# TaWeiTu/vp8

Hardware: NVIDIA B200
Metric: decoded 1080p frames/s (higher is better)
Workload: dtype u8

## Files before the change

vp8_b200/csrc/cuda/recon_kernels.cu:

```cuda
#include "recon_kernels.h"

#include <algorithm>
#include <cstring>

namespace vp8r {

__constant__ int c_taps[2][8][2];
__constant__ int c_taps6[2][8][6];
__constant__ unsigned short c_bpred_lut[10 * 16];

static int PackTaps(int a, int b, int c, int d) {
  return (a & 0xff) | ((b & 0xff) << 8) | ((c & 0xff) << 16) | ((d & 0xff) << 24);
}

static void BuildBpredLut(unsigned short *lut) {
  auto L = [](int k) { return 3 - k; };
  auto A = [](int k) { return 5 + k; };
  const int P = 4;
  auto put3 = [&](int mode, int y, int x, int a, int b, int c) {
    lut[mode * 16 + y * 4 + x] = (unsigned short)(a | (b << 4) | (c << 8) | (0 << 12));
  };
  auto put2 = [&](int mode, int y, int x, int a, int c) {
    lut[mode * 16 + y * 4 + x] = (unsigned short)(a | (a << 4) | (c << 8) | (1 << 12));
  };
// ... 20 lines not shown
  put3(7, 3, 3, A(5), A(6), A(7));
  put2(8, 3, 0, 0, 1);    put3(8, 3, 1, 0, 1, 2); put2(8, 2, 0, 1, 2);    put2(8, 3, 2, 1, 2);
  put3(8, 2, 1, 1, 2, 3); put3(8, 3, 3, 1, 2, 3); put2(8, 2, 2, 2, 3);    put2(8, 1, 0, 2, 3);
  put3(8, 2, 3, 2, 3, 4); put3(8, 1, 1, 2, 3, 4); put2(8, 1, 2, 3, 4);    put2(8, 0, 0, 3, 4);
  put3(8, 1, 3, 3, 4, 5); put3(8, 0, 1, 3, 4, 5); put3(8, 0, 2, 4, 5, 6); put3(8, 0, 3, 5, 6, 7);
  put2(9, 0, 0, L(0), L(1));       put3(9, 0, 1, L(0), L(1), L(2)); put2(9, 0, 2, L(1), L(2));
  put2(9, 1, 0, L(1), L(2));       put3(9, 0, 3, L(1), L(2), L(3)); put3(9, 1, 1, L(1), L(2), L(3));
  put2(9, 1, 2, L(2), L(3));       put2(9, 2, 0, L(2), L(3));       put3(9, 1, 3, L(2), L(3), L(3));
  put3(9, 2, 1, L(2), L(3), L(3));
  put3(9, 2, 2, L(3), L(3), L(3)); put3(9, 2, 3, L(3), L(3), L(3)); put3(9, 3, 0, L(3), L(3), L(3));
  put3(9, 3, 1, L(3), L(3), L(3)); put3(9, 3, 2, L(3), L(3), L(3)); put3(9, 3, 3, L(3), L(3), L(3));
}

cudaError_t InitKernelTables() {
  static const int six[8][6] = {{0, 0, 128, 0, 0, 0},  {0, -6, 123, 12, -1, 0},   {2, -11, 108, 36, -8, 1},
                                {0, -9, 93, 50, -6, 0}, {3, -16, 77, 77, -16, 3}, {0, -6, 50, 93, -9, 0},
                                {1, -8, 36, 108, -11, 2}, {0, -1, 12, 123, -6, 0}};
  int taps[2][8][2];
  for (int f = 0; f < 8; ++f) {
    taps[0][f][0] = PackTaps(six[f][0], six[f][1], six[f][2], six[f][3]);
    taps[0][f][1] = PackTaps(six[f][4], six[f][5], 0, 0);
    taps[1][f][0] = PackTaps(0, 0, 128 - 16 * f, 16 * f);
    taps[1][f][1] = 0;
  }
  cudaError_t err = cudaMemcpyToSymbol(c_taps, taps, sizeof(taps));
  if (err != cudaSuccess) return err;
  int taps6[2][8][6];
  for (int f = 0; f < 8; ++f)
    for (int k = 0; k < 6; ++k) {
      taps6[0][f][k] = six[f][k];
      taps6[1][f][k] = k == 2 ? 128 - 16 * f : (k == 3 ? 16 * f : 0);
    }
  err = cudaMemcpyToSymbol(c_taps6, taps6, sizeof(taps6));
  if (err != cudaSuccess) return err;
  err = InitParseTables();
  if (err != cudaSuccess) return err;
  unsigned short lut[160];
  std::memset(lut, 0, sizeof(lut));
  BuildBpredLut(lut);
  err = InitEncodeTables(lut);
  if (err != cudaSuccess) return err;
  return cudaMemcpyToSymbol(c_bpred_lut, lut, sizeof(lut));
}

__device__ __forceinline__ int dp4a_us(unsigned a, int b, int c) {
  int d;
  asm("dp4a.u32.s32 %0, %1, %2, %3;" : "=r"(d) : "r"(a), "r"(b), "r"(c));
  return d;
}
__device__ __forceinline__ int clamp255(int x) { return min(max(x, 0), 255); }
__device__ __forceinline__ int clamp128(int x) { return min(max(x, -128), 127); }
__device__ __forceinline__ int s16(int x) { return (int)(short)x; }

__device__ __forceinline__ void Idct4x4(int *m) {
#pragma unroll
  for (int i = 0; i < 4; ++i) {
    int a = m[i] + m[8 + i], b = m[i] - m[8 + i];
    int t1 = (m[4 + i] * 35468) >> 16;
    int t2 = m[12 + i] + ((m[12 + i] * 20091) >> 16);
    int c = t1 - t2;
    t1 = m[4 + i] + ((m[4 + i] * 20091) >> 16);
    t2 = (m[12 + i] * 35468) >> 16;
    int d = t1 + t2;
    m[i] = s16(a + d);
    m[12 + i] = s16(a - d);
    m[4 + i] = s16(b + c);
    m[8 + i] = s16(b - c);
  }
#pragma unroll
  for (int i = 0; i < 4; ++i) {
    int *r = m + 4 * i;
    int a = r[0] + r[2], b = r[0] - r[2];
    int t1 = (r[1] * 35468) >> 16;
    int t2 = r[3] + ((r[3] * 20091) >> 16);
    int c = t1 - t2;
    t1 = r[1] + ((r[1] * 20091) >> 16);
    t2 = (r[3] * 35468) >> 16;
    int d = t1 + t2;
    r[0] = s16((a + d + 4) >> 3);
    r[3] = s16((a - d + 4) >> 3);
    r[1] = s16((b + c + 4) >> 3);
    r[2] = s16((b - c + 4) >> 3);
  }
}

__device__ __forceinline__ void Iwht4x4(int *m) {
#pragma unroll
  for (int i = 0; i < 4; ++i) {
    int a = m[i] + m[12 + i], b = m[4 + i] + m[8 + i];
    int c = m[4 + i] - m[8 + i], d = m[i] - m[12 + i];
    m[i] = s16(a + b);
    m[4 + i] = s16(c + d);
    m[8 + i] = s16(a - b);
    m[12 + i] = s16(d - c);
  }
#pragma unroll
  for (int i = 0; i < 4; ++i) {
    int *r = m + 4 * i;
    int a = r[0] + r[3], b = r[1] + r[2];
    int c = r[1] - r[2], d = r[0] - r[3];
    r[0] = s16((a + b + 3) >> 3);
    r[1] = s16((c + d + 3) >> 3);
    r[2] = s16((a - b + 3) >> 3);
    r[3] = s16((d - c + 3) >> 3);
  }
}

__device__ __forceinline__ bool WarpResidual(const DevFrameJob &job, const vp8r_mb_info &mb, int lane,
                                            short *y2_slot, int *res) {
  const unsigned mask = mb.coef_mask;
  if (mask == 0) return false;
  const bool has_y2 = (mb.flags & VP8R_MB_HAS_Y2) != 0;
  const int blk = lane < 24 ? lane + 1 : 0;
  const bool coded = lane <= 24 && ((mask >> blk) & 1);
  const int16_t *dq = job.dq[(mb.flags >> VP8R_MB_QSEG_SHIFT) & 3];
#pragma unroll
  for (int i = 0; i < 16; ++i) res[i] = 0;
  if (coded) {
    const int at = __popc(mask & ((1u << blk) - 1));
    const int4 *src = reinterpret_cast<const int4 *>(job.payload + (size_t)(mb.coef_offset + at) * 16);
    int4 lo = __ldg(src), hi = __ldg(src + 1);
    int w[8] = {lo.x, lo.y, lo.z, lo.w, hi.x, hi.y, hi.z, hi.w};
    int dc = blk == 0 ? dq[VP8R_DQ_Y2_DC] : (blk <= 16 ? dq[VP8R_DQ_Y1_DC] : dq[VP8R_DQ_UV_DC]);
    int ac = blk == 0 ? dq[VP8R_DQ_Y2_AC] : (blk <= 16 ? dq[VP8R_DQ_Y1_AC] : dq[VP8R_DQ_UV_AC]);
#pragma unroll
    for (int i = 0; i < 8; ++i) {
      res[2 * i] = s16(s16(w[i]) * ac);
      res[2 * i + 1] = s16((w[i] >> 16) * ac);
    }
    res[0] = s16(s16(w[0]) * dc);
  }
  bool any = coded;
  if (has_y2 && (mask & 1)) {
    if (lane == 24) {
      Iwht4x4(res);
#pragma unroll
      for (int i = 0; i < 16; ++i) y2_slot[i] = (short)res[i];
    }
    __syncwarp();
    if (lane < 16) {
      res[0] = y2_slot[lane];
      any = true;
    }
    __syncwarp();
  }
  if (lane < 24 && any) Idct4x4(res);
  return lane < 24 && any;
}

__device__ __forceinline__ unsigned Filter4(unsigned lo, unsigned mid, unsigned hi, int t03, int t45) {
  unsigned out = 0;
#pragma unroll
  for (int j = 0; j < 4; ++j) {
    unsigned a = j ? __funnelshift_r(lo, mid, 8 * j) : lo;
    unsigned b = j ? __funnelshift_r(mid, hi, 8 * j) : mid;
    int s = dp4a_us(a, t03, 64);
    s = dp4a_us(b, t45, s);
    out |= (unsigned)clamp255(s >> 7) << (8 * j);
  }
  return out;
}

__device__ __forceinline__ void Transpose4x4(unsigned r0, unsigned r1, unsigned r2, unsigned r3, unsigned &c0,
                                             unsigned &c1, unsigned &c2, unsigned &c3) {
  unsigned t0 = __byte_perm(r0, r1, 0x5140), t1 = __byte_perm(r2, r3, 0x5140);
  unsigned t2 = __byte_perm(r0, r1, 0x7362), t3 = __byte_perm(r2, r3, 0x7362);
  c0 = __byte_perm(t0, t1, 0x5410);
  c1 = __byte_perm(t0, t1, 0x7632);
  c2 = __byte_perm(t2, t3, 0x5410);
  c3 = __byte_perm(t2, t3, 0x7632);
}

__device__ __forceinline__ unsigned PackSat4(int o0, int o1, int o2, int o3) {
  unsigned t, d;
  asm("cvt.pack.sat.u8.s32.b32 %0, %1, %2, %3;" : "=r"(t) : "r"(o3), "r"(o2), "r"(0));
  asm("cvt.pack.sat.u8.s32.b32 %0, %1, %2, %3;" : "=r"(d) : "r"(o1), "r"(o0), "r"(t));
  return d;
}

__device__ __forceinline__ unsigned Filter4P(unsigned lo, unsigned mid, unsigned hi, int t03, int t45) {
  int s[4];
#pragma unroll
  for (int j = 0; j < 4; ++j) {
    unsigned a = j ? __funnelshift_r(lo, mid, 8 * j) : lo;
    unsigned b = j ? __funnelshift_r(mid, hi, 8 * j) : mid;
    s[j] = dp4a_us(b, t45, dp4a_us(a, t03, 64)) >> 7;
  }
  return PackSat4(s[0], s[1], s[2], s[3]);
}

struct TapsAt {
  int lo1, lo2, lo3, mid1, mid2, mid3, hi3;
};
__device__ __forceinline__ TapsAt MakeTapsAt(int t03, int t45) {
  TapsAt t;
  t.lo1 = t03 << 8; t.lo2 = t03 << 16; t.lo3 = t03 << 24;
  t.mid1 = (int)__funnelshift_l((unsigned)t03, (unsigned)t45, 8);
  t.mid2 = (int)__funnelshift_l((unsigned)t03, (unsigned)t45, 16);
  t.mid3 = (int)__funnelshift_l((unsigned)t03, (unsigned)t45, 24);
  t.hi3 = (int)((unsigned)t45 >> 8);
  return t;
}
__device__ __forceinline__ unsigned Filter4T(unsigned lo, unsigned mid, unsigned hi, int t03, int t45, const TapsAt &t) {
  const int s0 = dp4a_us(mid, t45, dp4a_us(lo, t03, 64)) >> 7;
  const int s1 = dp4a_us(mid, t.mid1, dp4a_us(lo, t.lo1, 64)) >> 7;
  const int s2 = dp4a_us(mid, t.mid2, dp4a_us(lo, t.lo2, 64)) >> 7;
  const int s3 = dp4a_us(hi, t.hi3, dp4a_us(mid, t.mid3, dp4a_us(lo, t.lo3, 64))) >> 7;
  return PackSat4(s0, s1, s2, s3);
}

__device__ __forceinline__ unsigned Vert6(const unsigned *e, const unsigned *o, const int *t) {
  const unsigned bias = (8192u + 64u) * 0x00010001u;
  unsigned ae = bias, ao = bias;
#pragma unroll
  for (int k = 0; k < 6; ++k) {
    ae += (unsigned)t[k] * e[k];
    ao += (unsigned)t[k] * o[k];
  }
  ae = (ae >> 7) & 0x01ff01ffu;
  ao = (ao >> 7) & 0x01ff01ffu;
  ae = __vmins2(__viaddmax_s16x2(ae, 0xffc0ffc0u, 0u), 0x00ff00ffu);
  ao = __vmins2(__viaddmax_s16x2(ao, 0xffc0ffc0u, 0u), 0x00ff00ffu);
  return ae | (ao << 8);
// ... 23 lines not shown
      "MBAR_WAIT_%=:\n\t"
      "mbarrier.try_wait.parity.shared::cta.b64 p, [%0], %1;\n\t"
      "@p bra MBAR_DONE_%=;\n\t"
      "bra MBAR_WAIT_%=;\n\t"
      "MBAR_DONE_%=:\n\t}" ::"r"(SmemAddr(bar)), "r"(parity)
      : "memory");
}
__device__ __forceinline__ void TmaLoad2D(void *dst, const DevTensorMap *map, int x, int y, unsigned long long *bar) {
  asm volatile("cp.async.bulk.tensor.2d.shared::cluster.global.mbarrier::complete_tx::bytes [%0], [%1, {%2, %3}], [%4];" ::"r"(
                   SmemAddr(dst)),
               "l"(map), "r"(x), "r"(y), "r"(SmemAddr(bar))
               : "memory");
}

struct __align__(128) InterTile {
  unsigned char luma[kTmaLumaBoxH * kTmaLumaBoxW];
  unsigned char pad0[1024 - kTmaLumaBoxH * kTmaLumaBoxW];
  unsigned char cu[kTmaChromaBoxH * kTmaChromaBoxW];
  unsigned char pad1[640 - kTmaChromaBoxH * kTmaChromaBoxW];
  unsigned char cv[kTmaChromaBoxH * kTmaChromaBoxW];
  unsigned char pad2[640 - kTmaChromaBoxH * kTmaChromaBoxW - 8];
  unsigned long long bar;
};
static_assert(sizeof(InterTile) == 2304, "tile layout");
constexpr unsigned kInterTileTxBytes = kTmaLumaBoxH * kTmaLumaBoxW + 2 * kTmaChromaBoxH * kTmaChromaBoxW;

struct WholeMbGeometry {
  int fr, fc, cfr, cfc;
  int wy, wx, cwy, cwx;
};
__device__ __forceinline__ WholeMbGeometry WholeGeometry(const DevFrameJob &job, const vp8r_mb_info &mb, int mb_r, int mb_c) {
  WholeMbGeometry g;
  const int mvr = mb.mv[0], mvc = mb.mv[1];
  const int sr = s16(4 * mvr), sc = s16(4 * mvc);
  const int ar = (abs(sr) + 4) >> 3, ac = (abs(sc) + 4) >> 3;
  int cmr = sr < 0 ? -ar : ar, cmc = sc < 0 ? -ac : ac;
  if (job.version == 3) {
    cmr &= ~7;
    cmc &= ~7;
  }
  g.fr = mvr & 7; g.fc = mvc & 7; g.cfr = cmr & 7; g.cfc = cmc & 7;
  g.wy = min(max(mb_r * 16 + (mvr >> 3) - 2, -kBorder), job.mb_rows * 16 + kBorder - 21);
  g.wx = min(max(mb_c * 16 + (mvc >> 3) - 2, -kBorder), job.mb_cols * 16 + kBorder - 21);
  g.cwy = min(max(mb_r * 8 + (cmr >> 3) - 2, -kBorder), job.mb_rows * 8 + kBorder - 13);
  g.cwx = min(max(mb_c * 8 + (cmc >> 3) - 2, -kBorder), job.mb_cols * 8 + kBorder - 13);
  return g;
}

struct __align__(16) InterScratch {
  unsigned hl[23 * 4];
  unsigned hc[2][13 * 2];
  short res[24][16];
  short y2[16];
};

template <bool kTma>
__device__ __forceinline__ void InterMacroblockWhole(const DevFrameJob &job, const vp8r_mb_info &mb, int mb_r, int mb_c,
                                                     int lane, InterScratch &s, bool has_res, const WholeMbGeometry &g,
                                                     InterTile *tile) {
  const int ref_id = (mb.flags >> VP8R_MB_REF_SHIFT) & 3;
  const int bil = job.version != 0;
  const int fr = g.fr, fc = g.fc, cfr = g.cfr, cfc = g.cfc;

  if (kTma) {
    MbarWait(&tile->bar, 0);
    {
      const int dx = (g.wx + kBorder) & 15;
      const int w = lane & 3, row0 = lane >> 2, base = (dx >> 2) + w;
      const unsigned shift = (dx & 3) * 8;
      const int r_lo = fr ? 0 : 2, r_hi = (fr | fc) ? (fr ? 21 : 18) : 0;
      const int t03 = c_taps[bil][fc][0], t45 = c_taps[bil][fc][1];
      const TapsAt ta = MakeTapsAt(t03, t45);
#pragma unroll
      for (int k = 0; k < 3; ++k) {
        const int row = row0 + 8 * k;
        if (row >= r_lo && row < r_hi) {
          const unsigned *p = reinterpret_cast<const unsigned *>(tile->luma + row * kTmaLumaBoxW) + base;
          const unsigned w0 = p[0], w1 = p[1], w2 = p[2];
          const unsigned lo = __funnelshift_r(w0, w1, shift), mid = __funnelshift_r(w1, w2, shift), hi = w2 >> shift;
          s.hl[HlRow(row) + w] = fc ? Filter4T(lo, mid, hi, t03, t45, ta) : __funnelshift_r(lo, mid, 16);
        }
      }
    }
    {
      const int dx = (g.cwx + kBorder) & 15;
      const int row = lane >> 1, cw_ = lane & 1, base = (dx >> 2) + cw_;
      const unsigned shift = (dx & 3) * 8;
      const int r_lo = cfr ? 0 : 2, r_hi = (cfr | cfc) ? (cfr ? 13 : 10) : 0;
      const int t03 = c_taps[bil][cfc][0], t45 = c_taps[bil][cfc][1];
      const TapsAt ta = MakeTapsAt(t03, t45);
      if (row >= r_lo && row < r_hi) {
#pragma unroll
        for (int pl = 0; pl < 2; ++pl) {
          const unsigned *p = reinterpret_cast<const unsigned *>((pl ? tile->cv : tile->cu) + row * kTmaChromaBoxW) + base;
          const unsigned w0 = p[0], w1 = p[1], w2 = p[2];
          const unsigned lo = __funnelshift_r(w0, w1, shift), mid = __funnelshift_r(w1, w2, shift), hi = w2 >> shift;
          s.hc[pl][row * 2 + cw_] = cfc ? Filter4T(lo, mid, hi, t03, t45, ta) : __funnelshift_r(lo, mid, 16);
        }
      }
    }
  } else
  {
    const int pitch = job.pitch_y, cpitch = job.pitch_c;
    const int wy = g.wy, wx = g.wx;
    const uint8_t *wp = job.ref[ref_id].y + (ptrdiff_t)wy * pitch + wx;
    const unsigned shift = ((unsigned)(size_t)wp & 3u) * 8;
// ... 62 lines not shown
      out1 = Vert6(e + 1, o + 1, t);
    } else if (kTma && fc == 0) {
      const int dx2 = ((g.wx + kBorder) & 15) + 2;
      const unsigned *p = reinterpret_cast<const unsigned *>(tile->luma + (y0 + 2) * kTmaLumaBoxW) + (dx2 >> 2) + w;
      const unsigned sh = (dx2 & 3) * 8;
      out0 = __funnelshift_r(p[0], p[1], sh);
      out1 = __funnelshift_r(p[kTmaLumaBoxW / 4], p[kTmaLumaBoxW / 4 + 1], sh);
    } else {
      out0 = s.hl[HlRow(y0 + 2) + w];
      out1 = s.hl[HlRow(y0 + 3) + w];
    }
    if (has_res) {
      const uint2 *rp = reinterpret_cast<const uint2 *>(&s.res[(y0 >> 2) * 4 + w][(y0 & 3) * 4]);
      const uint2 ra = rp[0], rb = rp[1];
      out0 = AddResidual4(out0, ra.x, ra.y);
      out1 = AddResidual4(out1, rb.x, rb.y);
    }
    uint8_t *d = job.cur.y + (ptrdiff_t)(mb_r * 16 + y0) * job.pitch_y + mb_c * 16 + 4 * w;
    *reinterpret_cast<unsigned *>(d) = out0;
    *reinterpret_cast<unsigned *>(d + job.pitch_y) = out1;
  }
  {
    const int pl = lane >> 4, y = (lane >> 1) & 7, w = lane & 1;
    const unsigned *h = s.hc[pl];
    unsigned out;
    if (cfr) {
      unsigned e[6], o[6];
#pragma unroll
      for (int k = 0; k < 6; ++k) {
        const unsigned r = h[(y + k) * 2 + w];
        e[k] = __byte_perm(r, 0, 0x4240);
        o[k] = __byte_perm(r, 0, 0x4341);
      }
      out = Vert6(e, o, c_taps6[bil][cfr]);
    } else if (kTma && cfc == 0) {
      const int dx2 = ((g.cwx + kBorder) & 15) + 2;
      const unsigned *p = reinterpret_cast<const unsigned *>((pl ? tile->cv : tile->cu) + (y + 2) * kTmaChromaBoxW) + (dx2 >> 2) + w;
      out = __funnelshift_r(p[0], p[1], (dx2 & 3) * 8);
    } else {
      out = h[(y + 2) * 2 + w];
    }
    if (has_res) {
      const uint2 ra = *reinterpret_cast<const uint2 *>(&s.res[16 + pl * 4 + (y >> 2) * 2 + w][(y & 3) * 4]);
      out = AddResidual4(out, ra.x, ra.y);
    }
    uint8_t *d = (pl ? job.cur.v : job.cur.u) + (ptrdiff_t)(mb_r * 8 + y) * job.pitch_c + mb_c * 8 + 4 * w;
    *reinterpret_cast<unsigned *>(d) = out;
  }
}

constexpr int kInterWarps = 4;

#ifndef VP8R_INTER_MINBLOCKS
#define VP8R_INTER_MINBLOCKS 12
#endif
template <bool kTma>
__device__ __forceinline__ void InterOneMacroblock(const DevFrameJob &job, int mb_r, int mb_c, int lane, InterScratch &scratch, InterTile *tile) {
  const int mb_index = mb_r * job.mb_cols + mb_c;
  vp8r_mb_info mb;
  {
    const int4 *p = reinterpret_cast<const int4 *>(job.mbs + mb_index);
    int4 a = __ldg(p), b = __ldg(p + 1);
    mb.flags = a.x; mb.coef_mask = a.y; mb.coef_offset = a.z;
    mb.mv[0] = (short)(a.w & 0xffff); mb.mv[1] = (short)(a.w >> 16);
    mb.aux[0] = b.x; mb.aux[1] = b.y;
  }
  if (!(mb.flags & VP8R_MB_IS_INTER)) return;

  const bool split = ((mb.flags >> VP8R_MB_MODE_SHIFT) & 7) == 4;
  WholeMbGeometry geo{};
  if (!split) {
    geo = WholeGeometry(job, mb, mb_r, mb_c);
    if (kTma && lane == 0) {
      const DevTensorMap *maps = job.ref_tmap[(mb.flags >> VP8R_MB_REF_SHIFT) & 3];
      MbarExpectTx(&tile->bar, kInterTileTxBytes);
      TmaLoad2D(tile->luma, maps + 0, (geo.wx + kBorder) & ~15, geo.wy + kBorder, &tile->bar);
      TmaLoad2D(tile->cu, maps + 1, (geo.cwx + kBorder) & ~15, geo.cwy + kBorder, &tile->bar);
      TmaLoad2D(tile->cv, maps + 2, (geo.cwx + kBorder) & ~15, geo.cwy + kBorder, &tile->bar);
    }
  }
  int res[16];
  const bool has_res = WarpResidual(job, mb, lane, scratch.y2, res);
  if (!split) {
    const bool mb_has_res = mb.coef_mask != 0;
    if (mb_has_res && lane < 24) {
      uint4 *dst = reinterpret_cast<uint4 *>(scratch.res[lane]);
#pragma unroll
      for (int q = 0; q < 2; ++q) {
        unsigned v[4];
#pragma unroll
        for (int i = 0; i < 4; ++i) {
          const int a = has_res ? res[8 * q + 2 * i] : 0, b = has_res ? res[8 * q + 2 * i + 1] : 0;
          v[i] = ((unsigned)a & 0xffffu) | ((unsigned)b << 16);
        }
        dst[q] = make_uint4(v[0], v[1], v[2], v[3]);
      }
    }
    InterMacroblockWhole<kTma>(job, mb, mb_r, mb_c, lane, scratch, mb_has_res, geo, tile);
    return;
  }
  if (lane >= 24) return;

  const int ref_id = (mb.flags >> VP8R_MB_REF_SHIFT) & 3;
  const int *split_mv = reinterpret_cast<const int *>(job.payload + (size_t)mb.aux[0] * 16);

  int mvr, mvc, bx, by, pitch, plane_w, plane_h;
  const uint8_t *ref;
  uint8_t *dst;
  if (lane < 16) {
    int m = split ? __ldg(split_mv + lane) : (int)((unsigned short)mb.mv[0] | ((unsigned)(unsigned short)mb.mv[1] << 16));
    mvr = (short)(m & 0xffff);
    mvc = m >> 16;
    by = mb_r * 16 + (lane >> 2) * 4;
    bx = mb_c * 16 + (lane & 3) * 4;
    pitch = job.pitch_y;
    plane_w = job.mb_cols * 16;
    plane_h = job.mb_rows * 16;
    ref = job.ref[ref_id].y;
    dst = job.cur.y;
  } else {
    const int b = lane & 3, i = b >> 1, j = b & 1;
    int sr, sc;
    if (split) {
      const int k0 = i * 8 + j * 2;
      int m0 = __ldg(split_mv + k0), m1 = __ldg(split_mv + k0 + 1), m2 = __ldg(split_mv + k0 + 4),
          m3 = __ldg(split_mv + k0 + 5);
      sr = (short)(m0 & 0xffff) + (short)(m1 & 0xffff) + (short)(m2 & 0xffff) + (short)(m3 & 0xffff);
      sc = (m0 >> 16) + (m1 >> 16) + (m2 >> 16) + (m3 >> 16);
    } else {
      sr = 4 * mb.mv[0];
      sc = 4 * mb.mv[1];
    }
    sr = s16(sr);
    sc = s16(sc);
    mvr = (sr >= 0 ? (sr + 4) : (sr - 4)) / 8;
    mvc = (sc >= 0 ? (sc + 4) : (sc - 4)) / 8;
    if (job.version == 3) {
      mvr &= ~7;
      mvc &= ~7;
    }
    by = mb_r * 8 + i * 4;
    bx = mb_c * 8 + j * 4;
    pitch = job.pitch_c;
    plane_w = job.mb_cols * 8;
    plane_h = job.mb_rows * 8;
    ref = lane < 20 ? job.ref[ref_id].u : job.ref[ref_id].v;
    dst = lane < 20 ? job.cur.u : job.cur.v;
  }

  const int fr = mvr & 7, fc = mvc & 7;
  int wy = by + (mvr >> 3) - 2, wx = bx + (mvc >> 3) - 2;
  wy = min(max(wy, -kBorder), plane_h + kBorder - 9);
  wx = min(max(wx, -kBorder), plane_w + kBorder - 9);
  const uint8_t *wp = ref + (ptrdiff_t)wy * pitch + wx;
  const unsigned shift = ((unsigned)(size_t)wp & 3u) * 8;
  const unsigned *wrow = reinterpret_cast<const unsigned *>(wp - ((size_t)wp & 3));
  const int wpitch = pitch >> 2;

  unsigned out[4];
  if ((fr | fc) == 0) {
#pragma unroll
    for (int i = 0; i < 4; ++i) {
      const unsigned *p = wrow + (i + 2) * wpitch;
      unsigned w0 = p[0], w1 = p[1], w2 = p[2];
      unsigned lo = __funnelshift_r(w0, w1, shift), mid = __funnelshift_r(w1, w2, shift);
      out[i] = __funnelshift_r(lo, mid, 16);
    }
  } else {
    const int bil = job.version != 0;
    unsigned h[9];
    if (fc) {
      const int t03 = c_taps[bil][fc][0], t45 = c_taps[bil][fc][1];
#pragma unroll
      for (int i = 0; i < 9; ++i) {
        const unsigned *p = wrow + i * wpitch;
        unsigned w0 = p[0], w1 = p[1], w2 = p[2];
        unsigned lo = __funnelshift_r(w0, w1, shift), mid = __funnelshift_r(w1, w2, shift), hi = w2 >> shift;
        h[i] = Filter4(lo, mid, hi, t03, t45);
      }
    } else {
#pragma unroll
      for (int i = 0; i < 9; ++i) {
        const unsigned *p = wrow + i * wpitch;
        unsigned w0 = p[0], w1 = p[1], w2 = p[2];
        unsigned lo = __funnelshift_r(w0, w1, shift), mid = __funnelshift_r(w1, w2, shift);
        h[i] = __funnelshift_r(lo, mid, 16);
      }
    }
    if (fr) {
      const int t03 = c_taps[bil][fr][0], t45 = c_taps[bil][fr][1];
      unsigned a0, a1, a2, a3, b0, b1, b2, b3;
      Transpose4x4(h[0], h[1], h[2], h[3], a0, a1, a2, a3);
      Transpose4x4(h[4], h[5], h[6], h[7], b0, b1, b2, b3);
      unsigned c0 = Filter4(a0, b0, h[8], t03, t45);
      unsigned c1 = Filter4(a1, b1, h[8] >> 8, t03, t45);
      unsigned c2 = Filter4(a2, b2, h[8] >> 16, t03, t45);
      unsigned c3 = Filter4(a3, b3, h[8] >> 24, t03, t45);
      Transpose4x4(c0, c1, c2, c3, out[0], out[1], out[2], out[3]);
    } else {
      out[0] = h[2]; out[1] = h[3]; out[2] = h[4]; out[3] = h[5];
    }
  }

  uint8_t *d = dst + (ptrdiff_t)by * pitch + bx;
#pragma unroll
  for (int i = 0; i < 4; ++i) {
    unsigned v = out[i];
    if (has_res) {
      unsigned o = 0;
#pragma unroll
      for (int j = 0; j < 4; ++j) o |= (unsigned)clamp255(s16((int)((v >> (8 * j)) & 0xff) + res[i * 4 + j])) << (8 * j);
      v = o;
    }
    *reinterpret_cast<unsigned *>(d + (ptrdiff_t)i * pitch) = v;
  }
}

#ifndef VP8R_INTER_MBS_PER_WARP
#define VP8R_INTER_MBS_PER_WARP 1
#endif
constexpr int kInterMbsPerWarp = VP8R_INTER_MBS_PER_WARP;
template <bool kTma>
__global__ void __launch_bounds__(kInterWarps * 32, VP8R_INTER_MINBLOCKS) InterKernel(const DevFrameJob *__restrict__ jobs) {
  __shared__ InterScratch s_scratch[kInterWarps];
  __shared__ InterTile s_tile[kTma ? kInterWarps : 1];
  const DevFrameJob &job = jobs[blockIdx.z];
  const int warp = __shfl_sync(0xffffffffu, (int)(threadIdx.x >> 5), 0), lane = threadIdx.x & 31;
  const int mb_r = blockIdx.y, cols = job.mb_cols;
  const int first_c = (blockIdx.x * kInterWarps + warp) * kInterMbsPerWarp;
  if (mb_r >= job.mb_rows || first_c >= cols) return;
  if (JobFailed(job) || JobInter(job) == 0) return;
  if (kTma) {
    if (lane == 0) MbarInit(&s_tile[warp].bar, 1);
    __syncwarp();
  }
#pragma unroll 1
  for (int k = 0; k < kInterMbsPerWarp; ++k) {
    if (first_c + k >= cols) break;
    InterOneMacroblock<kTma>(job, mb_r, first_c + k, lane, s_scratch[warp], &s_tile[kTma ? warp : 0]);
    __syncwarp();
  }
}

cudaError_t LaunchInter(const DevFrameJob *jobs, int n_frames, int max_cols, int max_rows, cudaStream_t st, bool tma) {
  static_assert(kInterMbsPerWarp == 1, "the TMA path arms each warp's barrier once");
  const int per_cta = kInterWarps * kInterMbsPerWarp;
  if (max_rows > 65535 || n_frames > 65535) return cudaErrorInvalidValue;
  dim3 grid((max_cols + per_cta - 1) / per_cta, max_rows, n_frames);
  if (tma) InterKernel<true><<<grid, kInterWarps * 32, 0, st>>>(jobs);
  else InterKernel<false><<<grid, kInterWarps * 32, 0, st>>>(jobs);
  return cudaGetLastError();
}

constexpr int kWaveWarps = 32;

__device__ __forceinline__ void WaitRow(volatile int *progress, int row, int need) {
  if (row < 0) return;
  while (progress[row] < need) __nanosleep(40);
  __threadfence_block();
}
__device__ __forceinline__ void PublishRow(volatile int *progress, int row, int done, int lane) {
  __syncwarp();
  __threadfence_block();
  if (lane == 0) progress[row] = done;
}

struct __align__(16) IntraScratch {
  short y2[16];
  short res[24][16];
  unsigned char tile[17][24];
};

__device__ __forceinline__ void PredictMbBlock(const DevFrameJob &job, int mb_r, int mb_c, int lane, int ymode,
                                               int uvmode, bool do_luma, const short *res, bool has_res) {
  const bool luma = lane < 16;
  const int n4 = luma ? 4 : 2;
  const int first = luma ? 0 : (lane < 20 ? 16 : 20);
  const int b = lane - first, i = luma ? (b >> 2) : (b >> 1), j = luma ? (b & 3) : (b & 1);
  const int pitch = luma ? job.pitch_y : job.pitch_c;
  uint8_t *plane = luma ? job.cur.y : (lane < 20 ? job.cur.u : job.cur.v);
  const int n = luma ? 16 : 8;
  uint8_t *mbp = plane + (ptrdiff_t)(mb_r * n) * pitch + mb_c * n;
  const bool active = lane < 24 && (do_luma || !luma);
  const int mode = luma ? ymode : uvmode;
  const bool have_above = mb_r > 0, have_left = mb_c > 0;

  unsigned aw = 0x7f7f7f7fu;
  int l[4] = {129, 129, 129, 129};
  int P = have_above ? (have_left ? 0 : 129) : 127;
  if (lane < 24) {
    if (have_above) aw = *reinterpret_cast<const unsigned *>(mbp - pitch + 4 * j);
    if (have_left) {
#pragma unroll
      for (int k = 0; k < 4; ++k) l[k] = mbp[(ptrdiff_t)(4 * i + k) * pitch - 1];
    }
    if (have_above && have_left) P = mbp[-pitch - 1];
  }
  int sum_a = (int)__dp4a(aw, 0x01010101u, 0u);
  int sum_l = l[0] + l[1] + l[2] + l[3];
  int tot_a = 0, tot_l = 0;
#pragma unroll
  for (int k = 0; k < 4; ++k) {
    int va = __shfl_sync(0xffffffffu, sum_a, first + (k < n4 ? k : 0));
    int vl = __shfl_sync(0xffffffffu, sum_l, first + (k < n4 ? k * n4 : 0));
    if (k < n4) {
      tot_a += va;
      tot_l += vl;
    }
  }
  if (!active) return;

  unsigned rows[4];
  if (mode == 1) {
    rows[0] = rows[1] = rows[2] = rows[3] = aw;
  } else if (mode == 2) {
#pragma unroll
    for (int k = 0; k < 4; ++k) rows[k] = (unsigned)l[k] * 0x01010101u;
  } else if (mode == 0) {
    int v = 128;
    if (have_above || have_left) {
      int shf = (luma ? 3 : 2) + (have_above ? 1 : 0) + (have_left ? 1 : 0);
      int sum = (have_above ? tot_a : 0) + (have_left ? tot_l : 0);
      v = (sum + (1 << (shf - 1))) >> shf;
// ... 43 lines not shown
  if (lane < 16) s.tile[1 + lane][3] = (unsigned char)(mb_c == 0 ? 129 : mbp[(ptrdiff_t)lane * pitch - 1]);
  __syncwarp();

  const int py = (lane >> 2) & 3, px = lane & 3;
  for (int b = 0; b < 16; ++b) {
    const int i = b >> 2, j = b & 3;
    const int mode = (int)((mb.aux[b >> 3] >> ((b & 7) * 4)) & 15);
    int E = 0;
    if (lane < 4) {
      E = s.tile[1 + 4 * i + (3 - lane)][3 + 4 * j];
    } else if (lane < 9) {
      E = s.tile[4 * i][3 + 4 * j + (lane - 4)];
    } else if (lane < 13) {
      const int row = (j == 3) ? 0 : 4 * i;
      E = s.tile[row][3 + 4 * j + (lane - 4)];
    }
    const unsigned e = lut[mode * 16 + (lane & 15)];
    const int x0 = __shfl_sync(0xffffffffu, E, e & 15);
    const int x1 = __shfl_sync(0xffffffffu, E, (e >> 4) & 15);
    const int x2 = __shfl_sync(0xffffffffu, E, (e >> 8) & 15);
    const int dc_in = (lane < 4 || (lane >= 5 && lane < 9)) ? E : 0;
    const int dc = (__reduce_add_sync(0xffffffffu, dc_in) + 4) >> 3;
    const int kind = e >> 12;
    int v;
    if (kind == 0) v = (x0 + 2 * x1 + x2 + 2) >> 2;
    else if (kind == 1) v = (x0 + x2 + 1) >> 1;
    else if (kind == 2) v = dc;
    else v = clamp255(x0 + x1 - x2);
    if (lane < 16) {
      if ((res_mask >> b) & 1) v = clamp255(s16(v + s.res[b][lane]));
      s.tile[1 + 4 * i + py][4 + 4 * j + px] = (unsigned char)v;
    }
    __syncwarp();
  }
  if (lane < 16) {
    const unsigned *t = reinterpret_cast<const unsigned *>(&s.tile[1 + lane][4]);
    uint4 v = make_uint4(t[0], t[1], t[2], t[3]);
    *reinterpret_cast<uint4 *>(mbp + (ptrdiff_t)lane * pitch) = v;
  }
}

__device__ __forceinline__ void IntraMacroblock(const DevFrameJob &job, int r, int c, int lane, IntraScratch &s,
                                                const unsigned short *lut, volatile int *progress) {
  vp8r_mb_info mb;
  {
    const int4 *p = reinterpret_cast<const int4 *>(job.mbs + r * job.mb_cols + c);
    int4 a = __ldg(p), b = __ldg(p + 1);
    a.x = __shfl_sync(0xffffffffu, a.x, 0); a.y = __shfl_sync(0xffffffffu, a.y, 0);
    a.z = __shfl_sync(0xffffffffu, a.z, 0); a.w = __shfl_sync(0xffffffffu, a.w, 0);
    b.x = __shfl_sync(0xffffffffu, b.x, 0); b.y = __shfl_sync(0xffffffffu, b.y, 0);
    mb.flags = a.x; mb.coef_mask = a.y; mb.coef_offset = a.z;
    mb.aux[0] = b.x; mb.aux[1] = b.y;
  }
  int res[16];
  const bool has_res = WarpResidual(job, mb, lane, s.y2, res);
  const unsigned res_mask = __ballot_sync(0xffffffffu, has_res);
  if (lane < 24) {
#pragma unroll
    for (int i = 0; i < 16; ++i) s.res[lane][i] = (short)res[i];
  }
  if (progress) WaitRow(progress, r - 1, min(c + 2, job.mb_cols));
  __syncwarp();
  const int ymode = (mb.flags >> VP8R_MB_MODE_SHIFT) & 7, uvmode = (mb.flags >> VP8R_MB_UVMODE_SHIFT) & 3;
  PredictMbBlock(job, r, c, lane, ymode, uvmode, ymode != 4, lane < 24 ? s.res[lane] : s.res[0], has_res);
  if (ymode == 4) PredictBpred(job, r, c, lane, mb, s, res_mask, lut);
}

__global__ void __launch_bounds__(kWaveWarps * 32) IntraKernel(const DevFrameJob *__restrict__ jobs) {
  extern __shared__ __align__(16) unsigned char smem_raw[];
  const DevFrameJob &job = jobs[blockIdx.x];
  if (JobFailed(job) || JobIntra(job) == 0 || JobIntraLevels(job) != 0) return;
  const int rows = job.mb_rows, cols = job.mb_cols;
  volatile int *progress = reinterpret_cast<volatile int *>(smem_raw);
  unsigned short *lut = reinterpret_cast<unsigned short *>(smem_raw + ((rows * 4 + 15) & ~15));
  IntraScratch *scratch = reinterpret_cast<IntraScratch *>(reinterpret_cast<unsigned char *>(lut) + 320);
  for (int i = threadIdx.x; i < rows; i += blockDim.x) progress[i] = 0;
  for (int i = threadIdx.x; i < 160; i += blockDim.x) lut[i] = c_bpred_lut[i];
  __syncthreads();

  const int warp = __shfl_sync(0xffffffffu, (int)(threadIdx.x >> 5), 0), lane = threadIdx.x & 31;
  IntraScratch &s = scratch[warp];
  for (int r = warp; r < rows; r += kWaveWarps) {
    for (int c0 = 0; c0 < cols; c0 += 32) {
      unsigned flags = 0;
      if (c0 + lane < cols) flags = __ldg(&job.mbs[r * cols + c0 + lane].flags);
      unsigned intra_mask = __ballot_sync(0xffffffffu, (c0 + lane < cols) && !(flags & VP8R_MB_IS_INTER));
      while (intra_mask) {
        const int k = __ffs(intra_mask) - 1;
        intra_mask &= intra_mask - 1;
        const int c = c0 + k;
        IntraMacroblock(job, r, c, lane, s, lut, progress);
        PublishRow(progress, r, c + 1, lane);
      }
      PublishRow(progress, r, min(c0 + 32, cols), lane);
    }
  }
}

constexpr int kFlatWarps = 8;
__global__ void __launch_bounds__(kFlatWarps * 32) IntraFlatKernel(const DevFrameJob *__restrict__ jobs, int level) {
  __shared__ __align__(16) unsigned short lut[160];
  __shared__ IntraScratch scratch[kFlatWarps];
  const DevFrameJob &job = jobs[blockIdx.y];
  if (JobFailed(job) || job.dyn || job.levels_in_one_launch || level >= job.n_intra_levels) return;
  const unsigned first = __ldg(job.intra_levels + level), end = __ldg(job.intra_levels + level + 1);
  if (first + blockIdx.x * kFlatWarps >= end) return;
  for (int i = threadIdx.x; i < 160; i += blockDim.x) lut[i] = c_bpred_lut[i];
  __syncthreads();
  const int warp = __shfl_sync(0xffffffffu, (int)(threadIdx.x >> 5), 0), lane = threadIdx.x & 31;
  const unsigned slot = first + blockIdx.x * kFlatWarps + warp;
  if (slot >= end) return;
  const unsigned mb_index = __ldg(job.intra_levels + job.n_intra_levels + 1 + slot);
  const int r = mb_index / job.mb_cols, c = mb_index - r * job.mb_cols;
  IntraMacroblock(job, r, c, lane, scratch[warp], lut, nullptr);
}

constexpr int kLevelWarps = 16;
__global__ void __launch_bounds__(kLevelWarps * 32) IntraLevelsKernel(const DevFrameJob *__restrict__ jobs) {
  __shared__ __align__(16) unsigned short lut[160];
  __shared__ IntraScratch scratch[kLevelWarps];
  const DevFrameJob &job = jobs[blockIdx.x];
  if (JobFailed(job) || (!job.dyn && !job.levels_in_one_launch)) return;
  const int n_levels = JobIntraLevels(job);
  if (n_levels == 0) return;
  for (int i = threadIdx.x; i < 160; i += blockDim.x) lut[i] = c_bpred_lut[i];
  __syncthreads();
  const int warp = __shfl_sync(0xffffffffu, (int)(threadIdx.x >> 5), 0), lane = threadIdx.x & 31;
  const uint32_t *tab = JobLevelTable(job);
  const uint32_t *order = tab + n_levels + 1;
  for (int level = 0; level < n_levels; ++level) {
    const unsigned first = tab[level], end = tab[level + 1];
    for (unsigned slot = first + warp; slot < end; slot += kLevelWarps) {
      const unsigned mb_index = order[slot];
      const int r = mb_index / job.mb_cols, c = mb_index - r * job.mb_cols;
      IntraMacroblock(job, r, c, lane, scratch[warp], lut, nullptr);
    }
    __syncthreads();
  }
}

cudaError_t LaunchIntraLevels(const DevFrameJob *jobs, int n_frames, cudaStream_t st) {
  IntraLevelsKernel<<<n_frames, kLevelWarps * 32, 0, st>>>(jobs);
  return cudaGetLastError();
}

cudaError_t LaunchIntraFlat(const DevFrameJob *jobs, int n_frames, int level, int max_count, cudaStream_t st) {
  if (max_count <= 0) return cudaSuccess;
  dim3 grid((max_count + kFlatWarps - 1) / kFlatWarps, n_frames);
  IntraFlatKernel<<<grid, kFlatWarps * 32, 0, st>>>(jobs, level);
  return cudaGetLastError();
}

static size_t IntraSmemBytes(int max_rows) {
// ... 578 lines not shown
```

Baseline: 80180.

## Parallelize residual IDCT across lane quads and rework split-MV inter filtering

Replaces the per-lane whole-block IDCT/WHT with a 4-lanes-per-block column/row transform that goes through shared scratch. Only coded blocks are compacted and processed, eight at a time, and uncoded blocks are filled with DC-only or zero values. The split inter path now uses 8-byte aligned loads, a new horizontal Filter4T and a vertical Vert6 filter, and adds residuals from shared memory. Separately, inter min-blocks goes from 12 to 14 and the flat intra kernel gets a launch-bounds occupancy hint. The goal is less per-lane register pressure and skipping work on uncoded blocks, at the cost of extra warp syncs and shared-memory traffic.

```diff
diff --git a/vp8_b200/csrc/cuda/recon_kernels.cu b/vp8_b200/csrc/cuda/recon_kernels.cu
--- a/vp8_b200/csrc/cuda/recon_kernels.cu
+++ b/vp8_b200/csrc/cuda/recon_kernels.cu
@@ -96,123 +96,88 @@
 __device__ __forceinline__ int clamp128(int x) { return min(max(x, -128), 127); }
 __device__ __forceinline__ int s16(int x) { return (int)(short)x; }
 
-__device__ __forceinline__ void Idct4x4(int *m) {
-#pragma unroll
-  for (int i = 0; i < 4; ++i) {
-    int a = m[i] + m[8 + i], b = m[i] - m[8 + i];
-    int t1 = (m[4 + i] * 35468) >> 16;
-    int t2 = m[12 + i] + ((m[12 + i] * 20091) >> 16);
-    int c = t1 - t2;
-    t1 = m[4 + i] + ((m[4 + i] * 20091) >> 16);
-    t2 = (m[12 + i] * 35468) >> 16;
-    int d = t1 + t2;
-    m[i] = s16(a + d);
-    m[12 + i] = s16(a - d);
-    m[4 + i] = s16(b + c);
-    m[8 + i] = s16(b - c);
-  }
-#pragma unroll
-  for (int i = 0; i < 4; ++i) {
-    int *r = m + 4 * i;
-    int a = r[0] + r[2], b = r[0] - r[2];
-    int t1 = (r[1] * 35468) >> 16;
-    int t2 = r[3] + ((r[3] * 20091) >> 16);
-    int c = t1 - t2;
-    t1 = r[1] + ((r[1] * 20091) >> 16);
-    t2 = (r[3] * 35468) >> 16;
-    int d = t1 + t2;
-    r[0] = s16((a + d + 4) >> 3);
-    r[3] = s16((a - d + 4) >> 3);
-    r[1] = s16((b + c + 4) >> 3);
-    r[2] = s16((b - c + 4) >> 3);
-  }
-}
-
-__device__ __forceinline__ void Iwht4x4(int *m) {
-#pragma unroll
-  for (int i = 0; i < 4; ++i) {
-    int a = m[i] + m[12 + i], b = m[4 + i] + m[8 + i];
-    int c = m[4 + i] - m[8 + i], d = m[i] - m[12 + i];
-    m[i] = s16(a + b);
-    m[4 + i] = s16(c + d);
-    m[8 + i] = s16(a - b);
-    m[12 + i] = s16(d - c);
-  }
-#pragma unroll
-  for (int i = 0; i < 4; ++i) {
-    int *r = m + 4 * i;
-    int a = r[0] + r[3], b = r[1] + r[2];
-    int c = r[1] - r[2], d = r[0] - r[3];
-    r[0] = s16((a + b + 3) >> 3);
-    r[1] = s16((c + d + 3) >> 3);
-    r[2] = s16((a - b + 3) >> 3);
-    r[3] = s16((d - c + 3) >> 3);
-  }
-}
-
-__device__ __forceinline__ bool WarpResidual(const DevFrameJob &job, const vp8r_mb_info &mb, int lane,
-                                            short *y2_slot, int *res) {
+template <bool kRow>
+__device__ __forceinline__ void Idct1D(int *v) {
+  const int a = v[0] + v[2], b = v[0] - v[2];
+  const int c = ((v[1] * 35468) >> 16) - (v[3] + ((v[3] * 20091) >> 16));
+  const int d = (v[1] + ((v[1] * 20091) >> 16)) + ((v[3] * 35468) >> 16);
+  const int rnd = kRow ? 4 : 0, sh = kRow ? 3 : 0;
+  v[0] = s16((a + d + rnd) >> sh);
+  v[1] = s16((b + c + rnd) >> sh);
+  v[2] = s16((b - c + rnd) >> sh);
+  v[3] = s16((a - d + rnd) >> sh);
+}
+
+template <bool kRow>
+__device__ __forceinline__ void Iwht1D(int *v) {
+  const int a = v[0] + v[3], b = v[1] + v[2], c = v[1] - v[2], d = v[0] - v[3];
+  const int rnd = kRow ? 3 : 0, sh = kRow ? 3 : 0;
+  v[0] = s16((a + b + rnd) >> sh);
+  v[1] = s16((c + d + rnd) >> sh);
+  v[2] = s16((a - b + rnd) >> sh);
+  v[3] = s16((d - c + rnd) >> sh);
+}
+
+__device__ __forceinline__ void LoadColumn(const DevFrameJob &job, int at, int j, int dcq, int acq, int *v) {
+  const int4 *src = reinterpret_cast<const int4 *>(job.payload + (size_t)at * 16);
+  const int4 lo = __ldg(src), hi = __ldg(src + 1);
+  const bool odd = (j & 2) != 0;
+  const int w[4] = {odd ? lo.y : lo.x, odd ? lo.w : lo.z, odd ? hi.y : hi.x, odd ? hi.w : hi.z};
+  const int sh = (j & 1) * 16;
+#pragma unroll
+  for (int r = 0; r < 4; ++r) v[r] = s16(s16(w[r] >> sh) * (r == 0 && j == 0 ? dcq : acq));
+}
+
+template <bool kWht>
+__device__ __forceinline__ void Transform4Lanes(int *v, short *t, int j, bool active) {
+  if (kWht) Iwht1D<false>(v); else Idct1D<false>(v);
+  if (active) {
+#pragma unroll
+    for (int r = 0; r < 4; ++r) t[4 * r + j] = (short)v[r];
+  }
+  __syncwarp();
+  if (active) {
+    uint2 *row = reinterpret_cast<uint2 *>(t + 4 * j);
+    const uint2 p = *row;
+    v[0] = s16(p.x); v[1] = (int)p.x >> 16; v[2] = s16(p.y); v[3] = (int)p.y >> 16;
+    if (kWht) Iwht1D<true>(v); else Idct1D<true>(v);
+    *row = make_uint2(((unsigned)v[0] & 0xffffu) | ((unsigned)v[1] << 16), ((unsigned)v[2] & 0xffffu) | ((unsigned)v[3] << 16));
+  }
+}
+
+template <class Scratch>
+__device__ __forceinline__ void WarpResidual(const DevFrameJob &job, const vp8r_mb_info &mb, int lane, Scratch &s) {
   const unsigned mask = mb.coef_mask;
-  if (mask == 0) return false;
-  const bool has_y2 = (mb.flags & VP8R_MB_HAS_Y2) != 0;
-  const int blk = lane < 24 ? lane + 1 : 0;
-  const bool coded = lane <= 24 && ((mask >> blk) & 1);
+  const unsigned coded = (mask >> 1) & 0xffffffu;
+  const bool y2 = (mb.flags & VP8R_MB_HAS_Y2) && (mask & 1);
   const int16_t *dq = job.dq[(mb.flags >> VP8R_MB_QSEG_SHIFT) & 3];
-#pragma unroll
-  for (int i = 0; i < 16; ++i) res[i] = 0;
-  if (coded) {
-    const int at = __popc(mask & ((1u << blk) - 1));
-    const int4 *src = reinterpret_cast<const int4 *>(job.payload + (size_t)(mb.coef_offset + at) * 16);
-    int4 lo = __ldg(src), hi = __ldg(src + 1);
-    int w[8] = {lo.x, lo.y, lo.z, lo.w, hi.x, hi.y, hi.z, hi.w};
-    int dc = blk == 0 ? dq[VP8R_DQ_Y2_DC] : (blk <= 16 ? dq[VP8R_DQ_Y1_DC] : dq[VP8R_DQ_UV_DC]);
-    int ac = blk == 0 ? dq[VP8R_DQ_Y2_AC] : (blk <= 16 ? dq[VP8R_DQ_Y1_AC] : dq[VP8R_DQ_UV_AC]);
-#pragma unroll
-    for (int i = 0; i < 8; ++i) {
-      res[2 * i] = s16(s16(w[i]) * ac);
-      res[2 * i + 1] = s16((w[i] >> 16) * ac);
-    }
-    res[0] = s16(s16(w[0]) * dc);
-  }
-  bool any = coded;
-  if (has_y2 && (mask & 1)) {
-    if (lane == 24) {
-      Iwht4x4(res);
-#pragma unroll
-      for (int i = 0; i < 16; ++i) y2_slot[i] = (short)res[i];
-    }
+  const int g = lane >> 2, j = lane & 3;
+  if (y2) {
+    int v[4];
+    LoadColumn(job, mb.coef_offset, j, dq[VP8R_DQ_Y2_DC], dq[VP8R_DQ_Y2_AC], v);
+    Transform4Lanes<true>(v, s.y2, j, lane < 4);
     __syncwarp();
-    if (lane < 16) {
-      res[0] = y2_slot[lane];
-      any = true;
-    }
-    __syncwarp();
-  }
-  if (lane < 24 && any) Idct4x4(res);
-  return lane < 24 && any;
-}
-
-__device__ __forceinline__ unsigned Filter4(unsigned lo, unsigned mid, unsigned hi, int t03, int t45) {
-  unsigned out = 0;
-#pragma unroll
-  for (int j = 0; j < 4; ++j) {
-    unsigned a = j ? __funnelshift_r(lo, mid, 8 * j) : lo;
-    unsigned b = j ? __funnelshift_r(mid, hi, 8 * j) : mid;
-    int s = dp4a_us(a, t03, 64);
-    s = dp4a_us(b, t45, s);
-    out |= (unsigned)clamp255(s >> 7) << (8 * j);
-  }
-  return out;
-}
-
-__device__ __forceinline__ void Transpose4x4(unsigned r0, unsigned r1, unsigned r2, unsigned r3, unsigned &c0,
-                                             unsigned &c1, unsigned &c2, unsigned &c3) {
-  unsigned t0 = __byte_perm(r0, r1, 0x5140), t1 = __byte_perm(r2, r3, 0x5140);
-  unsigned t2 = __byte_perm(r0, r1, 0x7362), t3 = __byte_perm(r2, r3, 0x7362);
-  c0 = __byte_perm(t0, t1, 0x5410);
-  c1 = __byte_perm(t0, t1, 0x7632);
-  c2 = __byte_perm(t2, t3, 0x5410);
-  c3 = __byte_perm(t2, t3, 0x7632);
+  }
+  if (lane < 24 && ((coded >> lane) & 1)) s.order[__popc(coded & ((1u << lane) - 1))] = (unsigned char)lane;
+#pragma unroll
+  for (int c = lane; c < 48; c += 32) {
+    const int b = c >> 1;
+    if (!((coded >> b) & 1)) {
+      const unsigned v = y2 && b < 16 ? ((unsigned)((s.y2[b] + 4) >> 3) & 0xffffu) * 0x10001u : 0u;
+      reinterpret_cast<uint4 *>(s.res[b])[c & 1] = make_uint4(v, v, v, v);
+    }
+  }
+  __syncwarp();
+  const int n = __popc(coded);
+  for (int base = 0; base < n; base += 8) {
+    const int b = s.order[min(base + g, n - 1)];
+    const bool luma = b < 16;
+    int v[4];
+    LoadColumn(job, mb.coef_offset + __popc(mask & ((2u << b) - 1)), j, luma ? dq[VP8R_DQ_Y1_DC] : dq[VP8R_DQ_UV_DC],
+               luma ? dq[VP8R_DQ_Y1_AC] : dq[VP8R_DQ_UV_AC], v);
+    if (y2 && luma && j == 0) v[0] = s.y2[b];
+    Transform4Lanes<false>(v, s.res[b], j, base + g < n);
+  }
 }
 
 __device__ __forceinline__ unsigned PackSat4(int o0, int o1, int o2, int o3) {
@@ -342,6 +307,7 @@
   unsigned hc[2][13 * 2];
   short res[24][16];
   short y2[16];
+  unsigned char order[24];
 };
 
 template <bool kTma>
@@ -510,7 +476,7 @@
 constexpr int kInterWarps = 4;
 
 #ifndef VP8R_INTER_MINBLOCKS
-#define VP8R_INTER_MINBLOCKS 12
+#define VP8R_INTER_MINBLOCKS 14
 #endif
 template <bool kTma>
 __device__ __forceinline__ void InterOneMacroblock(const DevFrameJob &job, int mb_r, int mb_c, int lane, InterScratch &scratch, InterTile *tile) {
@@ -537,26 +503,13 @@
       TmaLoad2D(tile->cv, maps + 2, (geo.cwx + kBorder) & ~15, geo.cwy + kBorder, &tile->bar);
     }
   }
-  int res[16];
-  const bool has_res = WarpResidual(job, mb, lane, scratch.y2, res);
+  const bool has_res = mb.coef_mask != 0;
+  if (has_res) WarpResidual(job, mb, lane, scratch);
   if (!split) {
-    const bool mb_has_res = mb.coef_mask != 0;
-    if (mb_has_res && lane < 24) {
-      uint4 *dst = reinterpret_cast<uint4 *>(scratch.res[lane]);
-#pragma unroll
-      for (int q = 0; q < 2; ++q) {
-        unsigned v[4];
-#pragma unroll
-        for (int i = 0; i < 4; ++i) {
-          const int a = has_res ? res[8 * q + 2 * i] : 0, b = has_res ? res[8 * q + 2 * i + 1] : 0;
-          v[i] = ((unsigned)a & 0xffffu) | ((unsigned)b << 16);
-        }
-        dst[q] = make_uint4(v[0], v[1], v[2], v[3]);
-      }
-    }
-    InterMacroblockWhole<kTma>(job, mb, mb_r, mb_c, lane, scratch, mb_has_res, geo, tile);
+    InterMacroblockWhole<kTma>(job, mb, mb_r, mb_c, lane, scratch, has_res, geo, tile);
     return;
   }
+  __syncwarp();
   if (lane >= 24) return;
 
   const int ref_id = (mb.flags >> VP8R_MB_REF_SHIFT) & 3;
@@ -566,7 +519,7 @@
   const uint8_t *ref;
   uint8_t *dst;
   if (lane < 16) {
-    int m = split ? __ldg(split_mv + lane) : (int)((unsigned short)mb.mv[0] | ((unsigned)(unsigned short)mb.mv[1] << 16));
+    const int m = __ldg(split_mv + lane);
     mvr = (short)(m & 0xffff);
     mvc = m >> 16;
     by = mb_r * 16 + (lane >> 2) * 4;
@@ -578,19 +531,11 @@
     dst = job.cur.y;
   } else {
     const int b = lane & 3, i = b >> 1, j = b & 1;
-    int sr, sc;
-    if (split) {
-      const int k0 = i * 8 + j * 2;
-      int m0 = __ldg(split_mv + k0), m1 = __ldg(split_mv + k0 + 1), m2 = __ldg(split_mv + k0 + 4),
-          m3 = __ldg(split_mv + k0 + 5);
-      sr = (short)(m0 & 0xffff) + (short)(m1 & 0xffff) + (short)(m2 & 0xffff) + (short)(m3 & 0xffff);
-      sc = (m0 >> 16) + (m1 >> 16) + (m2 >> 16) + (m3 >> 16);
-    } else {
-      sr = 4 * mb.mv[0];
-      sc = 4 * mb.mv[1];
-    }
-    sr = s16(sr);
-    sc = s16(sc);
+    const int k0 = i * 8 + j * 2;
+    const int m0 = __ldg(split_mv + k0), m1 = __ldg(split_mv + k0 + 1), m2 = __ldg(split_mv + k0 + 4),
+              m3 = __ldg(split_mv + k0 + 5);
+    const int sr = s16((short)(m0 & 0xffff) + (short)(m1 & 0xffff) + (short)(m2 & 0xffff) + (short)(m3 & 0xffff));
+    const int sc = s16((m0 >> 16) + (m1 >> 16) + (m2 >> 16) + (m3 >> 16));
     mvr = (sr >= 0 ? (sr + 4) : (sr - 4)) / 8;
     mvc = (sc >= 0 ? (sc + 4) : (sc - 4)) / 8;
     if (job.version == 3) {
@@ -610,65 +555,51 @@
   int wy = by + (mvr >> 3) - 2, wx = bx + (mvc >> 3) - 2;
   wy = min(max(wy, -kBorder), plane_h + kBorder - 9);
   wx = min(max(wx, -kBorder), plane_w + kBorder - 9);
-  const uint8_t *wp = ref + (ptrdiff_t)wy * pitch + wx;
+  const uint8_t *__restrict__ wp = ref + (ptrdiff_t)wy * pitch + wx;
+  const uint2 *__restrict__ wrow = reinterpret_cast<const uint2 *>(wp - ((size_t)wp & 7));
+  const bool upper = ((size_t)wp & 4) != 0;
   const unsigned shift = ((unsigned)(size_t)wp & 3u) * 8;
-  const unsigned *wrow = reinterpret_cast<const unsigned *>(wp - ((size_t)wp & 3));
-  const int wpitch = pitch >> 2;
-
+  const int wpitch = pitch >> 3;
+
+  const int bil = job.version != 0;
+  const int r_lo = fr ? 0 : 2, r_hi = fr ? 9 : 6;
+  const int t03 = c_taps[bil][fc][0], t45 = c_taps[bil][fc][1];
+  const TapsAt ta = MakeTapsAt(t03, t45);
+  unsigned h[9];
+#pragma unroll
+  for (int i = 0; i < 9; ++i) {
+    if (i >= r_lo && i < r_hi) {
+      const uint2 a = __ldg(wrow + i * wpitch), b = __ldg(wrow + i * wpitch + 1);
+      const unsigned w0 = upper ? a.y : a.x, w1 = upper ? b.x : a.y, w2 = upper ? b.y : b.x;
+      const unsigned lo = __funnelshift_r(w0, w1, shift), mid = __funnelshift_r(w1, w2, shift), hi = w2 >> shift;
+      h[i] = fc ? Filter4T(lo, mid, hi, t03, t45, ta) : __funnelshift_r(lo, mid, 16);
+    }
+  }
   unsigned out[4];
-  if ((fr | fc) == 0) {
-#pragma unroll
-    for (int i = 0; i < 4; ++i) {
-      const unsigned *p = wrow + (i + 2) * wpitch;
-      unsigned w0 = p[0], w1 = p[1], w2 = p[2];
-      unsigned lo = __funnelshift_r(w0, w1, shift), mid = __funnelshift_r(w1, w2, shift);
-      out[i] = __funnelshift_r(lo, mid, 16);
-    }
+  if (fr) {
+    const int v03 = c_taps[bil][fr][0], v45 = c_taps[bil][fr][1];
+    const int t[6] = {(signed char)v03, (signed char)(v03 >> 8), (signed char)(v03 >> 16), v03 >> 24,
+                      (signed char)v45, (signed char)(v45 >> 8)};
+    unsigned e[9], o[9];
+#pragma unroll
+    for (int k = 0; k < 9; ++k) {
+      e[k] = __byte_perm(h[k], 0, 0x4240);
+      o[k] = __byte_perm(h[k], 0, 0x4341);
+    }
+#pragma unroll
+    for (int i = 0; i < 4; ++i) out[i] = Vert6(e + i, o + i, t);
   } else {
-    const int bil = job.version != 0;
-    unsigned h[9];
-    if (fc) {
-      const int t03 = c_taps[bil][fc][0], t45 = c_taps[bil][fc][1];
-#pragma unroll
-      for (int i = 0; i < 9; ++i) {
-        const unsigned *p = wrow + i * wpitch;
-        unsigned w0 = p[0], w1 = p[1], w2 = p[2];
-        unsigned lo = __funnelshift_r(w0, w1, shift), mid = __funnelshift_r(w1, w2, shift), hi = w2 >> shift;
-        h[i] = Filter4(lo, mid, hi, t03, t45);
-      }
-    } else {
-#pragma unroll
-      for (int i = 0; i < 9; ++i) {
-        const unsigned *p = wrow + i * wpitch;
-        unsigned w0 = p[0], w1 = p[1], w2 = p[2];
-        unsigned lo = __funnelshift_r(w0, w1, shift), mid = __funnelshift_r(w1, w2, shift);
-        h[i] = __funnelshift_r(lo, mid, 16);
-      }
-    }
-    if (fr) {
-      const int t03 = c_taps[bil][fr][0], t45 = c_taps[bil][fr][1];
-      unsigned a0, a1, a2, a3, b0, b1, b2, b3;
-      Transpose4x4(h[0], h[1], h[2], h[3], a0, a1, a2, a3);
-      Transpose4x4(h[4], h[5], h[6], h[7], b0, b1, b2, b3);
-      unsigned c0 = Filter4(a0, b0, h[8], t03, t45);
-      unsigned c1 = Filter4(a1, b1, h[8] >> 8, t03, t45);
-      unsigned c2 = Filter4(a2, b2, h[8] >> 16, t03, t45);
-      unsigned c3 = Filter4(a3, b3, h[8] >> 24, t03, t45);
-      Transpose4x4(c0, c1, c2, c3, out[0], out[1], out[2], out[3]);
-    } else {
-      out[0] = h[2]; out[1] = h[3]; out[2] = h[4]; out[3] = h[5];
-    }
-  }
-
+#pragma unroll
+    for (int i = 0; i < 4; ++i) out[i] = h[2 + i];
+  }
   uint8_t *d = dst + (ptrdiff_t)by * pitch + bx;
+  const uint2 *rp = reinterpret_cast<const uint2 *>(scratch.res[lane]);
 #pragma unroll
   for (int i = 0; i < 4; ++i) {
     unsigned v = out[i];
     if (has_res) {
-      unsigned o = 0;
-#pragma unroll
-      for (int j = 0; j < 4; ++j) o |= (unsigned)clamp255(s16((int)((v >> (8 * j)) & 0xff) + res[i * 4 + j])) << (8 * j);
-      v = o;
+      const uint2 r = rp[i];
+      v = AddResidual4(v, r.x, r.y);
     }
     *reinterpret_cast<unsigned *>(d + (ptrdiff_t)i * pitch) = v;
   }
@@ -727,6 +658,7 @@
   short y2[16];
   short res[24][16];
   unsigned char tile[17][24];
+  unsigned char order[24];
 };
 
 __device__ __forceinline__ void PredictMbBlock(const DevFrameJob &job, int mb_r, int mb_c, int lane, int ymode,
@@ -876,18 +808,13 @@
     mb.flags = a.x; mb.coef_mask = a.y; mb.coef_offset = a.z;
     mb.aux[0] = b.x; mb.aux[1] = b.y;
   }
-  int res[16];
-  const bool has_res = WarpResidual(job, mb, lane, s.y2, res);
-  const unsigned res_mask = __ballot_sync(0xffffffffu, has_res);
-  if (lane < 24) {
-#pragma unroll
-    for (int i = 0; i < 16; ++i) s.res[lane][i] = (short)res[i];
-  }
+  const bool has_res = mb.coef_mask != 0;
+  if (has_res) WarpResidual(job, mb, lane, s);
   if (progress) WaitRow(progress, r - 1, min(c + 2, job.mb_cols));
   __syncwarp();
   const int ymode = (mb.flags >> VP8R_MB_MODE_SHIFT) & 7, uvmode = (mb.flags >> VP8R_MB_UVMODE_SHIFT) & 3;
   PredictMbBlock(job, r, c, lane, ymode, uvmode, ymode != 4, lane < 24 ? s.res[lane] : s.res[0], has_res);
-  if (ymode == 4) PredictBpred(job, r, c, lane, mb, s, res_mask, lut);
+  if (ymode == 4) PredictBpred(job, r, c, lane, mb, s, mb.coef_mask >> 1, lut);
 }
 
 __global__ void __launch_bounds__(kWaveWarps * 32) IntraKernel(const DevFrameJob *__restrict__ jobs) {
@@ -922,7 +849,7 @@
 }
 
 constexpr int kFlatWarps = 8;
-__global__ void __launch_bounds__(kFlatWarps * 32) IntraFlatKernel(const DevFrameJob *__restrict__ jobs, int level) {
+__global__ void __launch_bounds__(kFlatWarps * 32, 8) IntraFlatKernel(const DevFrameJob *__restrict__ jobs, int level) {
   __shared__ __align__(16) unsigned short lut[160];
   __shared__ IntraScratch scratch[kFlatWarps];
   const DevFrameJob &job = jobs[blockIdx.y];
```

New measurement: 82640, median of 6. +3.1%, better.
